# sitzikbs/Nesti-Net

Measured on AMD Instinct MI355X. Metric: normals/sec (whole node), synthetic 100k-pt clouds, higher is better.
Workload: dtype f16x8c

## Files before the change

nesti-net_amd/csrc/conv.hip:

```cpp
#include <type_traits>

#include "kernels.h"
#include "mma.h"

namespace nesti {
namespace {

constexpr int kThreads = 512;
constexpr int kABytes = kTileM * kRowBytes;
constexpr int kPoolStride = 272;

__device__ __forceinline__ int vox2(int b) { return b < 4 ? b : 11 - b; }
__device__ __forceinline__ int tile_row(int remap, int log2S, int wave, int mi, int l) {
  if (!remap) return wave * 64 + mi * 32 + l;
  if (remap == 2) return ((mi * 32 + l) << 3) + vox2(wave);
  const int c = wave & 3, s = 2 * (wave >> 2) + mi;
  const int q = (c - s) & 3;
  if (log2S == 3) return ((2 * s + (l >> 4)) << 6) + ((2 * q + ((l >> 3) & 1)) << 3) + (l & 7);
  return ((l >> 2) << 6) + (s << 4) + (q << 2) + (l & 3);
}
struct SwzKey {
  int m_lo, m_hi;
  __device__ __forceinline__ SwzKey(int remap, int log2S) {
    const bool pts = remap && log2S == 2;
// ... 486 lines not shown
      }
#pragma unroll
      for (int it = 0; it < 2; ++it) {
        const int item = it * kThreads + tid;
        const int orow = item >> 4, cg = item & 15;
        const int pt_l = orow >> (log2V - 3), cell = orow & (Vo - 1);
        const int cz = cell >> (2 * log2So), cy = (cell >> log2So) & (So - 1), cx = cell & (So - 1);
        const int base = (pt_l << log2V) + ((((2 * cz) << log2S) + 2 * cy) << log2S) + 2 * cx;
        float4 m = make_float4(-INFINITY, -INFINITY, -INFINITY, -INFINITY);
#pragma unroll
        for (int a = 0; a < 8; ++a) {
          const int row = base + ((a >> 2) << (2 * log2S)) + (((a >> 1) & 1) << log2S) + (a & 1);
          const float4 v = *reinterpret_cast<const float4*>(smem + row * kPoolStride + cg * 16);
          m.x = fmaxf(m.x, v.x); m.y = fmaxf(m.y, v.y); m.z = fmaxf(m.z, v.z); m.w = fmaxf(m.w, v.w);
        }
        const long long go = (r0 >> 3) + orow;
        if (go < (total_rows >> 3))
          store_out4<DT>(mp_b, go * p.mp_cstride, out_col0 + nh * 64 + cg * 4, m, out_esz, p.split);
      }
      __syncthreads();
    };
    mp_half(std::integral_constant<int, 0>{});
    if constexpr (TN == 128) mp_half(std::integral_constant<int, 1>{});
    return;
  }

  unsigned char* scratch = smem + wave * (32 * kPoolStride);
#pragma unroll
  for (int mi = 0; mi < 2; ++mi) {
#pragma unroll
    for (int nh = 0; nh < TN / 64; ++nh) {
#pragma unroll
      for (int n2 = 0; n2 < 2; ++n2) {
        const int ni = nh * 2 + n2;
        const int col = n2 * 32 + (lane & 31);
        const float bv = bias[ni * 32 + (lane & 31)];
#pragma unroll
        for (int r = 0; r < 16; ++r) {
          const int row = (r & 3) + 8 * (r >> 2) + 4 * khalf;
          *reinterpret_cast<float*>(scratch + row * kPoolStride + col * 4) = fmaxf(fmaf(acc[mi][ni][r], p.acc_scale, bv), act_floor);
        }
      }
      if (out_esz == 4) {
#pragma unroll
        for (int it = 0; it < 8; ++it) {
          const int row = it * 4 + (lane >> 4), cpos = lane & 15;
          const uint4 v = *reinterpret_cast<const uint4*>(scratch + row * kPoolStride + cpos * 16);
          const long long gr = r0 + tile_row(remap, log2S, wave, mi, row);
          if (gr < total_rows)
            *reinterpret_cast<uint4*>(out_b + (gr * p.out_cstride + out_col0 + nh * 64) * 4 + cpos * 16) = v;
        }
      } else {
        using E = Elem<DT == NESTI_F32 ? NESTI_BF16 : DT>;
#pragma unroll
        for (int it = 0; it < 4; ++it) {
          const int row = it * 8 + (lane >> 3), cpos = lane & 7;
          const float4 f0 = *reinterpret_cast<const float4*>(scratch + row * kPoolStride + cpos * 32);
          const float4 f1 = *reinterpret_cast<const float4*>(scratch + row * kPoolStride + cpos * 32 + 16);
          const long long gr = r0 + tile_row(remap, log2S, wave, mi, row);
          if (gr < total_rows) {
            store_act8<E>(out_b, gr * p.out_cstride, out_col0 + nh * 64 + cpos * 8, f0, f1, p.split);
            if (p.aux8_out && !second && p.x8_fmt != 6)
              store_aux8_8(reinterpret_cast<unsigned char*>(p.aux8_out) + gr * p.aux8_stride, n_local * TN + nh * 64 + cpos * 8, f0, f1,
                           aux_mul_lo, aux_mul_hi);
          }
        }
        if (p.aux8_out && !second && p.x8_fmt == 6) {
#pragma unroll
          for (int it = 0; it < 2; ++it) {
            const int row = it * 16 + (lane >> 2), c16 = lane & 3;
            const unsigned char* src = scratch + row * kPoolStride + c16 * 64;
            const long long gr = r0 + tile_row(remap, log2S, wave, mi, row);
            if (gr < total_rows)
              store_aux6_16(reinterpret_cast<unsigned char*>(p.aux8_out) + gr * p.aux8_stride, n_local * TN + nh * 64 + c16 * 16,
                            *reinterpret_cast<const float4*>(src), *reinterpret_cast<const float4*>(src + 16),
                            *reinterpret_cast<const float4*>(src + 32), *reinterpret_cast<const float4*>(src + 48));
          }
        }
      }
    }
  }
}

template <int DT, int TN, bool KPIPE, bool X3, bool WALK, bool X2 = false>
__global__ __launch_bounds__(kThreads) void conv_igemm_kernel(const ConvParams p) {
  if constexpr (!WALK) {
    conv_igemm_tile<DT, TN, KPIPE, X3, X2>(p, blockIdx.x, threadIdx.x);
  } else {
    const long long rows = (long long)live_points(p) << (3 * p.log2S);
    const unsigned m_live = (unsigned)((rows + kTileM - 1) / kTileM);
    const unsigned n_blocks = tile_rows8(m_live) * (unsigned)p.n_tiles;
    for (unsigned bid = blockIdx.x; bid < n_blocks; bid += gridDim.x) conv_igemm_tile<DT, TN, KPIPE, X3, X2>(p, bid, walk_trip(bid));
  }
}

template <int TN, bool KPIPE>
constexpr int lds_bytes() {
  constexpr size_t kPoolTile = (size_t)kTileM * kPoolStride + 16;
  constexpr size_t loop = KPIPE ? (size_t)2 * kABytes + 2 * TN * kRowBytes
                                : (size_t)kABytes + 4 * TN * kRowBytes + kRowBytes;
  static_assert(loop <= 163840 && kPoolTile <= 163840, "LDS budget");
  return (int)(loop > kPoolTile ? loop : kPoolTile);
}

template <int DT, int TN, bool KPIPE, bool X3>
int launch_one(const ConvParams& p, hipStream_t stream) {
  return launch_tiles<conv_igemm_kernel<DT, TN, KPIPE, X3, false>, conv_igemm_kernel<DT, TN, KPIPE, X3, true>>(
      p, lds_bytes<TN, KPIPE>(), kThreads, tile_rows8(p.m_tiles) * p.n_tiles, stream);
}
template <int DT, int TN>
int launch_one_x2(const ConvParams& p, hipStream_t stream) {
  return launch_tile_kernel<conv_igemm_kernel<DT, TN, true, false, false, true>>(p, lds_bytes<TN, true>(), kThreads,
                                                                                 tile_rows8(p.m_tiles) * p.n_tiles, stream);
}

template <int DT>
int launch_dt(const ConvParams& p, int TN, hipStream_t stream) {
  const bool kpipe = (p.n_taps == 1);
  if constexpr (DT != NESTI_F32) {
    if (p.x2) {
      if (!kpipe || p.x3native || p.walk) NESTI_FAIL("launch_conv: x2 is the filter pass's 1x1x1 / FC variant");
      if (TN == 128) return launch_one_x2<DT, 128>(p, stream);
      if (TN == 64) return launch_one_x2<DT, 64>(p, stream);
      NESTI_FAIL("launch_conv: unsupported N tile");
    }
    if (p.x3native) {
      if (TN == 128) return kpipe ? launch_one<DT, 128, true, true>(p, stream) : launch_one<DT, 128, false, true>(p, stream);
      if (TN == 64) return kpipe ? launch_one<DT, 64, true, true>(p, stream) : launch_one<DT, 64, false, true>(p, stream);
      NESTI_FAIL("launch_conv: unsupported N tile");
    }
  }
  if (p.x3native || p.x2) NESTI_FAIL("launch_conv: the pair / exact-weight K loops are for the 16-bit kernels");
  if (TN == 128) return kpipe ? launch_one<DT, 128, true, false>(p, stream) : launch_one<DT, 128, false, false>(p, stream);
  if (TN == 64) return kpipe ? launch_one<DT, 64, true, false>(p, stream) : launch_one<DT, 64, false, false>(p, stream);
  NESTI_FAIL("launch_conv: unsupported N tile");
}

}

int launch_conv(const ConvParams& p, int dtype, int TN, hipStream_t stream) {
  if (p.m_tiles <= 0 || p.n_tiles <= 0) return 0;
  if (p.pool_k > 1 && p.n_taps != 1) NESTI_FAIL("launch_conv: fused pooling needs a 1x1x1 layer");
  if (p.mp_mode != 0 && (p.log2S < 1 || !p.mp_out)) NESTI_FAIL("launch_conv: fused max-pool needs a volume >= 2^3 and an output");
  if (p.s_real && !(p.s_real == 3 && p.log2S == 2)) NESTI_FAIL("launch_conv: s_real is the 3^3 grid inside a 4^3 index space only");
  if (p.s_real && p.pool_k == 3) NESTI_FAIL("launch_conv: fused 3^3 avg-pool is not built for the embedded 3^3 volume");
  if (p.s_real && (p.mp_mode != 0 || p.mp_mode2 != 0)) NESTI_FAIL("launch_conv: the fused 2^3 max-pool does not apply to the 3^3 volume");
  if (p.mp_mode2 != 0 && (p.pool_k <= 1 || !p.mp_out || p.log2S < 1)) NESTI_FAIL("launch_conv: mp_mode2 belongs to a fused avg-pool half with a pooled output");
  if (p.pool_k > 1 && !((p.log2S == 3 && p.pool_k == 3) || (p.log2S == 2 && (p.pool_k == 2 || p.pool_k == 3)) ||
                        (p.log2S == 1 && p.pool_k == 2)))
    NESTI_FAIL("launch_conv: fused pooling supports (S,k) in {(8,3),(4,3),(4,2),(2,2)}");
  return with_elem_type(dtype, "launch_conv", [&](auto dt) { return launch_dt<decltype(dt)::value>(p, TN, stream); });
}

}
```

nesti-net_amd/csrc/kernels.h:

```cpp
#pragma once
#include <algorithm>
#include <type_traits>

#include "common.h"

namespace nesti {

constexpr unsigned kWalkGrid = 1024;

int launch_conv(const ConvParams& p, int dtype, int TN, hipStream_t stream);
int launch_conv8n(const ConvParams& p, int dtype, int k, hipStream_t stream);
int launch_conv4n(const ConvParams& p, int dtype, int k, hipStream_t stream);
int conv8_selftest();

__host__ __device__ __forceinline__ unsigned tile_rows8(unsigned m_tiles) { return (m_tiles + 7) / 8 * 8; }
template <class Params>
__device__ __forceinline__ int live_points(const Params& p) {
  int npts = p.npoints;
  if (p.npoints_ptr) npts = min(npts, *p.npoints_ptr);
  return npts;
}
struct TileId {
  int sub, m_tile;
};
__device__ __forceinline__ TileId tile_id(const unsigned bid, const int per_m) {
  const int xcd = bid & 7, grp = bid >> 3;
  return {grp % per_m, (grp / per_m) * 8 + xcd};
}
__device__ __forceinline__ int walk_trip(const unsigned bid) {
  if (bid != blockIdx.x) __syncthreads();
  int tid = threadIdx.x;
  asm volatile("" : "+v"(tid));
  return tid;
}

constexpr int kTapThreads = 512;
constexpr int kEpiStride = 144;
inline int check_tap_launch(const ConvParams& p, const char* who) {
  const std::string w(who);
  if (p.point_index) NESTI_FAIL(w + ": no input gather (k^3 layers never read the routed MuPS tensor)");
  if (p.pool_k > 1 || p.split_tile != p.n_tiles) NESTI_FAIL(w + ": no fused avg-pool / merged layers");
  if (p.mp_mode == 2) NESTI_FAIL(w + ": max-pool mode 2 is conv1's (a 1x1x1 layer)");
  if (p.mp_mode != 0 && !p.mp_out) NESTI_FAIL(w + ": fused max-pool needs an output");
  return 0;
}

template <auto Kernel>
int launch_tile_kernel(const ConvParams& p, int lds, unsigned threads, unsigned grid, hipStream_t stream) {
  constexpr int kMaxDevices = 64;
  static bool attr_set[kMaxDevices] = {};
  int dev = 0;
  NESTI_CHECK_HIP(hipGetDevice(&dev));
  if (dev < 0 || dev >= kMaxDevices || !attr_set[dev]) {
    NESTI_CHECK_HIP(hipFuncSetAttribute(reinterpret_cast<const void*>(Kernel), hipFuncAttributeMaxDynamicSharedMemorySize, lds));
    if (dev >= 0 && dev < kMaxDevices) attr_set[dev] = true;
  }
  hipLaunchKernelGGL(Kernel, dim3(grid), dim3(threads), lds, stream, p);
  NESTI_CHECK_HIP(hipGetLastError());
  return 0;
}
template <auto Kernel, auto WalkKernel>
int launch_tiles(const ConvParams& p, int lds, unsigned threads, unsigned n_blocks, hipStream_t stream) {
  if (!p.walk) return launch_tile_kernel<Kernel>(p, lds, threads, n_blocks, stream);
  return launch_tile_kernel<WalkKernel>(p, lds, threads, std::min(n_blocks, p.walk > 1 ? (unsigned)p.walk : kWalkGrid), stream);
}
template <class F>
int with_elem_type(int dtype, const char* who, F&& f) {
  if (dtype == NESTI_BF16) return f(std::integral_constant<int, NESTI_BF16>{});
  if (dtype == NESTI_F16) return f(std::integral_constant<int, NESTI_F16>{});
  if (dtype == NESTI_F32) return f(std::integral_constant<int, NESTI_F32>{});
  NESTI_FAIL(std::string(who) + ": unsupported dtype");
}

int launch_maxpool2(const PoolParams& p, int dtype, hipStream_t stream);
int launch_maxpool3s2(const PoolParams& p, int dtype, hipStream_t stream);

int launch_gate_finish(const float* logits, int lstride, int B, int E, float* probs,
                       int32_t* expert, int32_t* counts ,
                       int32_t* lists , hipStream_t stream);
constexpr int kMaxCascadeRounds = 24;
constexpr int kRoundCountsOff = 8, kTauEffOff = 40, kWidenUpperOff = 41, kWidenCountOff = 48, kWidenRoundsOff = 56;
static_assert(kRoundCountsOff + kMaxCascadeRounds <= kTauEffOff && kWidenRoundsOff + kMaxCascadeRounds <= 128, "fcounts layout");
int launch_gate_flag(const float* logits, int lstride, int B, int E, float tau, float widen, float* probs, int32_t* expert,
                     float* keep, int32_t* fcounts, int32_t* flag_list, int cap, int n_rounds, unsigned long long* cstat,
                     const unsigned long long* rstat, hipStream_t stream);
int launch_gate_widen(const float* keep, int B, int E, float widen, int32_t* fcounts, int32_t* flag_list, int cap, int n_rounds,
                      unsigned long long* cstat, hipStream_t stream);
int launch_gate_recheck(const float* logits, int lstride, const int32_t* flag_list, const int32_t* count_ptr, int cap, int E,
                        const float* keep, float* probs, int32_t* expert, unsigned long long* cstat, const int32_t* fcounts,
                        float widen, unsigned long long* rstat, hipStream_t stream);
int launch_stat_max_export(const unsigned long long* word, float* dst, hipStream_t stream);
int launch_stat_max_import(unsigned long long* word, const float* src, int n, hipStream_t stream);
int launch_round_counts(const int32_t* counts, int n_lists, int cap, int n_rounds, int32_t* out, hipStream_t stream);
// ... 18 lines not shown
```

nesti-net_amd/csrc/model.hip:

```cpp
#include <math.h>
#include <string.h>

#include <algorithm>
#include <map>
#include <memory>
#include <mutex>
#include <string>
#include <vector>

#include "kernels.h"
#include "plan.h"

#ifndef NESTI_GUARD_WALK_GRID
#define NESTI_GUARD_WALK_GRID 64
#endif
#ifndef NESTI_GUARD_LANES
#define NESTI_GUARD_LANES 2
#endif
#ifndef NESTI_GATE_WIDEN_WALK_GRID
#define NESTI_GATE_WIDEN_WALK_GRID 1
#endif
#ifndef NESTI_GUARD_WIDEN_WALK_GRID
#define NESTI_GUARD_WIDEN_WALK_GRID 8
#endif

namespace nesti {

static thread_local std::string g_error;
static bool g_experiment_mix = false;
void set_error(const std::string& msg) { g_error = msg; }

constexpr int kProfSlots = NESTI_PROF_PHASES * NESTI_PROF_CATEGORIES;
struct ProfState {
  bool on = false;
  int phase = NESTI_PHASE_INPUT;
  std::vector<hipEvent_t> pool;
  std::vector<std::pair<hipEvent_t, hipEvent_t>> spans[kProfSlots];
  double ms[kProfSlots] = {0};
  long long launches[kProfSlots] = {0};
};
static ProfState g_prof;
static std::mutex g_prof_mu;

static hipEvent_t prof_event() {
  if (!g_prof.pool.empty()) { hipEvent_t e = g_prof.pool.back(); g_prof.pool.pop_back(); return e; }
  hipEvent_t e = nullptr;
  (void)hipEventCreate(&e);
  return e;
}
static bool prof_capturing(hipStream_t st) {
  hipStreamCaptureStatus cs = hipStreamCaptureStatusNone;
  if (hipStreamIsCapturing(st, &cs) != hipSuccess) { (void)hipGetLastError(); return false; }
  return cs != hipStreamCaptureStatusNone;
}
void prof_phase(int phase) { if (g_prof.on) g_prof.phase = phase; }
int prof_begin(int cat, hipStream_t st) {
  if (!g_prof.on || prof_capturing(st)) return -1;
  std::lock_guard<std::mutex> lk(g_prof_mu);
  const int phase = (cat == NESTI_PROF_MUPS || cat == NESTI_PROF_PATCHES) ? NESTI_PHASE_INPUT : g_prof.phase;
  const int slot = phase * NESTI_PROF_CATEGORIES + cat;
  if (g_prof.spans[slot].size() >= (1u << 20)) return -1;
  hipEvent_t a = prof_event(), b = prof_event();
  (void)hipEventRecord(a, st);
  g_prof.spans[slot].push_back({a, b});
  return (slot << 20) | ((int)g_prof.spans[slot].size() - 1);
}
void prof_end(int, int token, hipStream_t st) {
  if (token < 0) return;
  std::lock_guard<std::mutex> lk(g_prof_mu);
  const int slot = token >> 20, idx = token & ((1 << 20) - 1);
  if (slot < kProfSlots && idx < (int)g_prof.spans[slot].size()) (void)hipEventRecord(g_prof.spans[slot][idx].second, st);
}
static void prof_collect() {
  std::lock_guard<std::mutex> lk(g_prof_mu);
  for (int c = 0; c < kProfSlots; ++c) {
    for (auto& sp : g_prof.spans[c]) {
      (void)hipEventSynchronize(sp.second);
      float ms = 0.f;
      if (hipEventElapsedTime(&ms, sp.first, sp.second) == hipSuccess) g_prof.ms[c] += ms;
      g_prof.launches[c] += 1;
      g_prof.pool.push_back(sp.first);
      g_prof.pool.push_back(sp.second);
    }
    g_prof.spans[c].clear();
  }
}

namespace {

struct PackedLayer : PackMeta {
  void* wpk = nullptr;
  float* bias = nullptr;
};

int upload(const PackedImage& img, PackedLayer* pl) {
  static_cast<PackMeta&>(*pl) = img;
  NESTI_CHECK_HIP(hipMalloc(&pl->wpk, img.w.size()));
  NESTI_CHECK_HIP(hipMemcpy(pl->wpk, img.w.data(), img.w.size(), hipMemcpyHostToDevice));
  NESTI_CHECK_HIP(hipMalloc((void**)&pl->bias, img.bias.size() * sizeof(float)));
  NESTI_CHECK_HIP(hipMemcpy(pl->bias, img.bias.data(), img.bias.size() * sizeof(float), hipMemcpyHostToDevice));
  return 0;
}

struct StatBlock {
  unsigned long long* dev = nullptr;
  StatBlock() = default;
  StatBlock(const StatBlock&) = delete;
  StatBlock& operator=(const StatBlock&) = delete;
  ~StatBlock() { if (dev) (void)hipFree(dev); }
  explicit operator bool() const { return dev != nullptr; }
  int alloc() { NESTI_CHECK_HIP(hipMalloc((void**)&dev, 64)); return reset(); }
  int reset() const { NESTI_CHECK_HIP(hipMemset(dev, 0, 64)); return 0; }
  int read(unsigned long long (&h)[8], int then_reset) const {
    memset(h, 0, sizeof(h));
    if (dev) NESTI_CHECK_HIP(hipMemcpy(h, dev, sizeof(h), hipMemcpyDeviceToHost));
    return dev && then_reset ? reset() : 0;
  }
};

}
}

struct nesti_model {
  nesti::Graph graph;
  int dtype = NESTI_BF16;
  std::map<std::pair<int, int>, nesti::PackedLayer> packed;
  const nesti::PackedLayer* packing(int form, int layer) const {
    auto it = packed.find({nesti::form_packing(form), layer});
    return it == packed.end() ? nullptr : &it->second;
  }
  const nesti::PackedLayer& main_packing(int layer) const {
    return *packing(nesti::act_planes(dtype) > 1 ? NESTI_DEBUG_FORM_PAIR : NESTI_DEBUG_FORM_PLAIN, layer);
  }
  bool cascade = false;
  nesti::Mode mode() const { return {graph, dtype, cascade}; }
  bool has_mix = false;
  int expert_mix = 0;
  int x8_mask = 0;
  int x8_fmt = 6;
  float x8_guard_thr = NESTI_X8_GUARD_DEFAULT;
  int x8_guard_walk = NESTI_GUARD_WALK_GRID;
  nesti::StatBlock gstat;
  static constexpr int kGuardLanes = NESTI_GUARD_LANES;
  struct GuardLane {
    hipStream_t gstream = nullptr;
    hipEvent_t gev_done[NESTI_MAX_EXPERTS] = {}, gev_join = nullptr;
    hipStream_t owner = nullptr;
    bool owned = false;
    std::mutex gmu;
  };
  mutable GuardLane glane[kGuardLanes];
  mutable std::mutex glane_mu;
  GuardLane* guard_lane(hipStream_t caller) const {
    std::lock_guard<std::mutex> lk(glane_mu);
    for (int i = 0; i < kGuardLanes; ++i) if (glane[i].owned && glane[i].owner == caller) return &glane[i];
    for (int i = 0; i < kGuardLanes; ++i) if (!glane[i].owned) { glane[i].owned = true; glane[i].owner = caller; return &glane[i]; }
    return &glane[0];
  }
  int gate_mix = 0;
  float tau = 0.25f;
  nesti::StatBlock cstat;
  bool reproducible = false;
  nesti::StatBlock rstat;
  unsigned long long* frozen() const { return reproducible ? rstat.dev : nullptr; }
  ~nesti_model() {
    for (auto& p : packed) {
      if (p.second.wpk) (void)hipFree(p.second.wpk);
      if (p.second.bias) (void)hipFree(p.second.bias);
    }
    for (auto& gl : glane) {
      if (gl.gstream) (void)hipStreamDestroy(gl.gstream);
      for (auto& ev : gl.gev_done) if (ev) (void)hipEventDestroy(ev);
      if (gl.gev_join) (void)hipEventDestroy(gl.gev_join);
    }
  }
};

namespace nesti {
namespace {

struct RunCtx {
  const nesti_model* m;
  Pass pass;
  int NB;
  const int32_t* npoints_ptr;
  const int32_t* point_index;
  hipStream_t stream;
  int walk;
};
RunCtx pass_ctx(const nesti_model* m, int tower, bool fast, int x8_mask, int NB, const int32_t* npoints_ptr, const int32_t* point_index,
                hipStream_t stream, int walk) {
  Pass ps;
  ps.tower = tower; ps.fast = fast; ps.x8_mask = x8_mask; ps.x8_fmt = m->x8_fmt;
  if (tower >= 0) ps.mix = m->expert_mix;
  else if (!m->cascade && m->gate_mix) { ps.mix = 1 << kGateMixBit; ps.zero_lo = m->gate_mix == 2; }
  return RunCtx{m, ps, NB, npoints_ptr, point_index, stream, walk};
}

int tower_ptrs(const RunCtx& rc, const Tower& T, const void* X0, unsigned char* ws, size_t ws_bytes, std::vector<unsigned char*>* ptr) {
  ptr->assign(T.bufs.size(), nullptr);
  (*ptr)[0] = (unsigned char*)X0;
  const Placement P = place_tower(T, rc.NB, pass_dtype(rc.pass.fast, rc.m->dtype));
  for (size_t i = 1; i < T.bufs.size(); ++i) (*ptr)[i] = ws + P.off[i];
  if (P.total > ws_bytes) NESTI_FAIL("workspace too small for this batch");
  return 0;
}

int run_op(const RunCtx& rc, const Tower& T, const Op& op, const std::vector<unsigned char*>& ptr) {
  const nesti_model* m = rc.m;
  const OpPlan plan = plan_op(m->graph, T, op, rc.pass, m->dtype);
  if (op.kind != Op::CONV) {
    PoolParams p = pool_params(T, op, plan, rc.NB);
    p.in = ptr[op.in_buf]; p.out = ptr[op.out_buf]; p.npoints_ptr = rc.npoints_ptr;
    const int tok = prof_begin(NESTI_PROF_POOL, rc.stream);
    const int rcp = op.kind == Op::MAX3 ? launch_maxpool3s2(p, plan.elem, rc.stream) : launch_maxpool2(p, plan.elem, rc.stream);
    prof_end(NESTI_PROF_POOL, tok, rc.stream);
    return rcp ? 1 : 0;
  }
  const LayerDesc& d = m->graph.layers[op.layer];
  const PackedLayer* pk = m->packing(plan.form.form, op.layer);
  if (!pk || pk->kind != plan.form.family)
    NESTI_FAIL("internal: layer " + d.scope + " is not packed for form " + std::to_string(plan.form.form) + " of this pass");
  ConvParams p = conv_params(m->graph, T, op, rc.pass, plan, *pk, plan.x8_sc_layer >= 0 ? m->main_packing(plan.x8_sc_layer).x8_sc : 0, rc.NB);
  p.in = ptr[op.in_buf]; p.out = ptr[op.out_buf]; p.wpk = pk->wpk; p.bias = pk->bias;
  p.npoints_ptr = rc.npoints_ptr; p.point_index = op.in_buf < 1 ? rc.point_index : nullptr;
  if (op.mp_buf >= 0) p.mp_out = ptr[op.mp_buf];
  if (p.x8) p.aux8_in = ptr[op.aux_in_buf];
  if (plan.form.producer) p.aux8_out = ptr[op.aux_out_buf];
  p.walk = rc.walk;
  const int cat = conv_category(d, *pk);
  const int tok = prof_begin(cat, rc.stream);
  const int rcv = pk->kind == 2   ? launch_conv8n(p, plan.elem, d.k, rc.stream)
                  : pk->kind == 3 ? launch_conv4n(p, plan.elem, d.k, rc.stream)
                                  : launch_conv(p, plan.elem, pk->TN, rc.stream);
  prof_end(cat, tok, rc.stream);
  return rcv ? 1 : 0;
}

int run_tower(const RunCtx& rc, const Tower& T, const void* X0, unsigned char* ws, size_t ws_bytes, float** out) {
  std::vector<unsigned char*> ptr;
  if (tower_ptrs(rc, T, X0, ws, ws_bytes, &ptr)) return 1;
  for (const Op& op : T.ops)
    if (run_op(rc, T, op, ptr)) return 1;
  *out = reinterpret_cast<float*>(ptr[T.out_buf]);
  return 0;
}

struct Arena {
  unsigned char* ws;
  int NB;
  WsLayout L;
  Arena(const nesti_model* m, void* ws_dev, int NB) : ws((unsigned char*)ws_dev), NB(NB), L(ws_layout(m->mode(), NB)) {}
  template <class T> T* at(size_t off) const { return reinterpret_cast<T*>(ws + off); }
  unsigned char* tower() const { return ws + L.tower; }
  size_t tower_size() const { return L.total - L.tower; }
};

int gate_cascade(const nesti_model* m, const void* X0, int B, const Arena& A, float* probs, int32_t* expert, int32_t* counts,
                 int32_t* lists, hipStream_t stream) {
  const int E = m->graph.cfg.n_experts;
  if (!expert) expert = A.at<int32_t>(A.L.expert);
  float* keep = A.at<float>(A.L.keep);
  int32_t* flag_list = A.at<int32_t>(A.L.flags);
  int32_t* fcounts = A.at<int32_t>(A.L.fcounts);
  const int lstride = m->graph.gate.bufs[m->graph.gate.out_buf].C;
  float* logits = nullptr;
  const RunCtx fast = pass_ctx(m, -1, true, 0, B, nullptr, nullptr, stream, 0);
  prof_phase(NESTI_PHASE_GATE);
  if (run_tower(fast, m->graph.gate, X0, A.tower(), A.tower_size(), &logits)) return 1;
  prof_phase(NESTI_PHASE_RECHECK);
  const int cap = std::min(cascade_cap(A.NB), B), rounds = (B + cap - 1) / cap;
  unsigned long long* rstat = m->frozen();
  if (launch_gate_flag(logits, lstride, B, E, m->tau, NESTI_GATE_WIDEN, probs, expert, keep, fcounts, flag_list, cap, rounds,
                       m->cstat.dev, rstat, stream))
    return 1;
  for (int pass = 0; pass <= (rstat ? 0 : NESTI_GATE_WIDEN_PASSES); ++pass) {
    if (pass >= 1 && launch_gate_widen(keep, B, E, NESTI_GATE_WIDEN, fcounts, flag_list, cap, rounds, m->cstat.dev, stream)) return 1;
    const int32_t* round_counts = fcounts + (pass == 0 ? kRoundCountsOff : kWidenRoundsOff);
    for (int r = 0; r < rounds; ++r) {
      const RunCtx exact = pass_ctx(m, -1, false, 0, cap, round_counts + r, flag_list + (size_t)r * cap, stream,
                                    pass >= 1 ? NESTI_GATE_WIDEN_WALK_GRID : r >= 1 ? 1 : 0);
      if (run_tower(exact, m->graph.gate, X0, A.tower(), A.tower_size(), &logits)) return 1;
      if (launch_gate_recheck(logits, lstride, flag_list + (size_t)r * cap, round_counts + r, cap, E, keep, probs, expert,
                              m->cstat.dev, fcounts, NESTI_GATE_WIDEN, rstat, stream))
        return 1;
    }
  }
  if (counts) return launch_route(expert, B, E, counts, lists, stream);
  return 0;
}

int gate_impl(const nesti_model* m, const void* X0, int B, const Arena& A, float* probs, int32_t* expert, int32_t* counts,
              int32_t* lists, hipStream_t stream) {
  if (m->cascade) return gate_cascade(m, X0, B, A, probs, expert, counts, lists, stream);
  const RunCtx rc = pass_ctx(m, -1, false, 0, B, nullptr, nullptr, stream, 0);
  float* logits = nullptr;
  prof_phase(NESTI_PHASE_GATE);
  if (run_tower(rc, m->graph.gate, X0, A.tower(), A.tower_size(), &logits)) return 1;
  const int lstride = m->graph.gate.bufs[m->graph.gate.out_buf].C;
  if (m->graph.cfg.arch == NESTI_ARCH_SWITCH)
    return launch_switch_finish(logits, lstride, B, 0.015f, probs, expert, counts, lists, stream);
  return launch_gate_finish(logits, lstride, B, m->graph.cfg.n_experts, probs, expert, counts, lists, stream);
}

constexpr int kGuardCountOff = 128, kGuardSlotOff = 140;
int experts_impl(const nesti_model* m, const void* X0, int B, const Arena& A, const int32_t* counts, const int32_t* lists, float* normals,
                 hipStream_t stream) {
  int32_t* ecounts = A.at<int32_t>(A.L.ecounts);
  int32_t* glist = m->graph.x8 ? A.at<int32_t>(A.L.glist) : nullptr;
  const int E = m->graph.cfg.n_experts;
  const int cap = std::min(expert_cap(A.NB), B), rounds = (B + cap - 1) / cap;
  prof_phase(NESTI_PHASE_EXPERTS);
  if (counts && launch_round_counts(counts, E, cap, rounds, ecounts, stream)) return 1;
  const size_t x0_row = mups_row_bytes(m->mode());
  const bool guard = counts && glist && m->x8_mask && m->gstat && m->x8_guard_thr >= 0.f;
  const int gcap = std::min(guard_cap(A.NB), B);
  float* gslot = guard ? reinterpret_cast<float*>(ecounts + kGuardSlotOff) : nullptr;
// ... 26 lines not shown
      float* out = nullptr;
      if (counts) {
        const int32_t* list = lists + (size_t)e * B + (size_t)r * cap;
        const int32_t* cnt = ecounts + e * rounds + r;
        const RunCtx rc = pass_ctx(m, e, false, m->x8_mask, cap, cnt, list, stream, r >= 1);
        if (run_tower(rc, T, X0, A.tower(), A.tower_size(), &out)) return 1;
        if (launch_scatter3(out, ostride, list, cnt, cap, normals, stream)) return 1;
      } else {
        const int take = std::min(cap, B - r * cap);
        const RunCtx rc = pass_ctx(m, e, false, m->x8_mask, take, nullptr, nullptr, stream, 0);
        if (run_tower(rc, T, (const unsigned char*)X0 + (size_t)r * cap * x0_row, A.tower(), A.tower_size(), &out)) return 1;
        if (launch_scatter3(out, ostride, nullptr, nullptr, take, normals + ((size_t)e * B + (size_t)r * cap) * 3, stream)) return 1;
      }
    }
    if (guard) {
      prof_phase(NESTI_PHASE_GUARD);
      if (side) {
        NESTI_CHECK_HIP(hipEventRecord(lane->gev_done[e], stream));
        NESTI_CHECK_HIP(hipStreamWaitEvent(lane->gstream, lane->gev_done[e], 0));
        if (guard_expert(e, lane->gstream, A.tower() + main_bytes, A.tower_size() - main_bytes, m->x8_guard_walk)) return 1;
      } else if (guard_expert(e, stream, A.tower(), A.tower_size(), m->x8_guard_walk)) {
        return 1;
      }
      prof_phase(NESTI_PHASE_EXPERTS);
    }
  }
  if (guard) {
    if (side) {
      NESTI_CHECK_HIP(hipEventRecord(lane->gev_join, lane->gstream));
      NESTI_CHECK_HIP(hipStreamWaitEvent(stream, lane->gev_join, 0));
      glk.unlock();
    }
    prof_phase(NESTI_PHASE_GUARD);
    for (int pass = 1; pass <= (rstat ? 0 : NESTI_X8_GUARD_WIDEN_PASSES); ++pass) {
      if (launch_x8_guard_begin(pass, m->x8_guard_thr, gscale, B, m->gstat.dev, gslot, nullptr, stream)) return 1;
      for (int e = 0; e < E; ++e)
        if (guard_expert(e, stream, A.tower(), A.tower_size(), NESTI_GUARD_WIDEN_WALK_GRID)) return 1;
    }
  }
  return 0;
}

}
}

using namespace nesti;

extern "C" {

const char* nesti_last_error(void) { return g_error.c_str(); }
const char* nesti_version(void) {
  return "nesti-hip 0.6 (gfx950)"
#ifdef NESTI_ATTRIBUTION
         " [measurement build: NESTI_ATTRIBUTION]"
#endif
#ifdef NESTI_EXPERIMENT_XW
         " [measurement build: NESTI_EXPERIMENT_XW]"
#endif
      ;
}

int nesti_mups_forward(const nesti_config_t* cfg, const float* points_dev, const int32_t* n_eff_dev, int B,
                       void* out_dev, int out_dtype, int out_cstride, void* stream) {
  if (B <= 0) return 0;
  if (!cfg || !points_dev || !n_eff_dev || !out_dev) NESTI_FAIL("nesti_mups_forward: null argument");
  const int tok = prof_begin(NESTI_PROF_MUPS, (hipStream_t)stream);
  const int rc = launch_mups(cfg, points_dev, n_eff_dev, B, out_dev, out_dtype, out_cstride, 0, (hipStream_t)stream);
  prof_end(NESTI_PROF_MUPS, tok, (hipStream_t)stream);
  return rc;
}

int nesti_model_create(const nesti_config_t* cfg, const nesti_tensor_t* tensors, int n_tensors, int dtype,
                       nesti_model_t** out) {
  if (!cfg || !tensors || !out) NESTI_FAIL("nesti_model_create: null argument");
  if (dtype != NESTI_F32 && dtype != NESTI_BF16 && dtype != NESTI_F16 && dtype != NESTI_BF16X3 && dtype != NESTI_F16X3 &&
      dtype != NESTI_F16X3C && dtype != NESTI_F16X8 && dtype != NESTI_F16X8C)
    NESTI_FAIL("nesti_model_create: bad dtype");
  if (dtype_cascade(dtype) && cfg->arch != NESTI_ARCH_EXPERTS)
    NESTI_FAIL("nesti_model_create: NESTI_F16X3C / NESTI_F16X8C is the two-stage gate of experts_n_est; use NESTI_F16X3 for the other models");
  if (dtype_x8(dtype) && (cfg->arch != NESTI_ARCH_EXPERTS || cfg->grid_n != 8))
    NESTI_FAIL("nesti_model_create: NESTI_F16X8 / NESTI_F16X8C (FP8 cross terms in the expert towers) is for experts_n_est on the 8^3 grid");
  std::unique_ptr<nesti_model> m(new nesti_model());
  m->cascade = dtype_cascade(dtype);
  const bool x8 = dtype_x8(dtype);
  dtype = main_dtype(dtype);
  m->dtype = dtype;
  if (build_graph(cfg, &m->graph, x8)) return 1;
  const TensorTable tt = tensor_table(tensors, n_tensors);
  bool any_conv8 = false;
  for (const LayerDesc& d : m->graph.layers) any_conv8 = any_conv8 || layer_kind(d, dtype) == 2;
  if (any_conv8 && conv8_selftest()) return 1;
  m->has_mix = g_experiment_mix && act_planes(dtype) > 1 && cfg->arch == NESTI_ARCH_EXPERTS && cfg->grid_n == 8;
  for (int t = -1; t < (int)m->graph.experts.size(); ++t) {
    std::vector<Pass> passes(1);
    if (m->cascade && t < 0) { passes.push_back(Pass()); passes.back().fast = true; }
    for (int fmt : {8, 6})
      if (x8 && t >= 0) { passes.push_back(Pass()); passes.back().x8_mask = 0xF; passes.back().x8_fmt = fmt; }
    if (m->has_mix) { passes.push_back(Pass()); passes.back().mix = t < 0 ? 1 << kGateMixBit : 0x3F; }
    for (Pass& ps : passes) {
      ps.tower = t;
      for (const Op& op : m->graph.tower(t).ops) {
        if (op.kind != Op::CONV) continue;
        const LayerDesc& d = m->graph.layers[op.layer];
        const LaunchForm f = launch_form(m->graph, op, ps, dtype);
        const int packing = form_packing(f.form);
        PackedLayer& pl = m->packed[{packing, op.layer}];
        PackedImage img;
        if (!pl.wpk && (pack_form(d, tt, packing, dtype, &img) || upload(img, &pl))) return 1;
        if (f.producer) pl.x8_sc = x8_activation_exponent(d, tt);
      }
    }
  }
  if (x8) {
    m->x8_mask = 0xF;
    if (m->gstat.alloc()) return 1;
    for (auto& gl : m->glane) {
      NESTI_CHECK_HIP(hipStreamCreateWithFlags(&gl.gstream, hipStreamNonBlocking));
      NESTI_CHECK_HIP(hipEventCreateWithFlags(&gl.gev_join, hipEventDisableTiming));
      for (int e = 0; e < cfg->n_experts; ++e) NESTI_CHECK_HIP(hipEventCreateWithFlags(&gl.gev_done[e], hipEventDisableTiming));
    }
  }
  if (m->cascade && m->cstat.alloc()) return 1;
  if ((m->cstat || m->gstat) && m->rstat.alloc()) return 1;
  NESTI_CHECK_HIP(hipDeviceSynchronize());
  *out = m.release();
  return 0;
}

void nesti_model_destroy(nesti_model_t* m) { delete m; }

int nesti_model_set_gate_margin(nesti_model_t* m, float tau) {
  if (!m || !m->cascade) NESTI_FAIL("nesti_model_set_gate_margin: not a NESTI_F16X3C model");
  if (!(tau >= 0.f)) NESTI_FAIL("nesti_model_set_gate_margin: tau must be >= 0");
  m->tau = tau;
  return 0;
}

int nesti_experiment_mix_enable(int on) {
  g_experiment_mix = on != 0;
  return 0;
}

int nesti_model_set_expert_mix(nesti_model_t* m, int mask) {
  if (!m) NESTI_FAIL("nesti_model_set_expert_mix: null model");
  if (mask && !m->has_mix) NESTI_FAIL("nesti_model_set_expert_mix: pair-mode experts_n_est models (8^3 grid) created after nesti_experiment_mix_enable(1) only");
  if (mask < 0 || mask >= (1 << 6)) NESTI_FAIL("nesti_model_set_expert_mix: mask has six bits");
  m->expert_mix = mask;
  return 0;
}

int nesti_model_set_x8_layers(nesti_model_t* m, int mask) {
  if (!m) NESTI_FAIL("nesti_model_set_x8_layers: null model");
  if (!m->graph.x8) NESTI_FAIL("nesti_model_set_x8_layers: not an NESTI_F16X8 / NESTI_F16X8C model");
  if (mask < 0 || mask > 0xF) NESTI_FAIL("nesti_model_set_x8_layers: mask has four bits (inception1 conv2 / conv3, inception2 conv2 / conv3)");
  m->x8_mask = mask;
  return 0;
}

int nesti_model_set_x8_format(nesti_model_t* m, int bits) {
  if (!m) NESTI_FAIL("nesti_model_set_x8_format: null model");
  if (!m->graph.x8) NESTI_FAIL("nesti_model_set_x8_format: not an NESTI_F16X8 / NESTI_F16X8C model");
  if (bits != 8 && bits != 6) NESTI_FAIL("nesti_model_set_x8_format: 8 (e4m3, one scale per layer) or 6 (e2m3, one scale per 16-channel block)");
  m->x8_fmt = bits;
  return 0;
}

// ... 458 lines not shown
```

Measured before the change: 51450.

## Add wide-N x3 pair conv kernel with 128x256 tiles and triple-buffered A

```diff
diff --git a/nesti-net_amd/csrc/conv.hip b/nesti-net_amd/csrc/conv.hip
--- a/nesti-net_amd/csrc/conv.hip
+++ b/nesti-net_amd/csrc/conv.hip
@@ -592,6 +592,300 @@
   }
 }
 
+constexpr int kWideRows = kTileM / 2;
+constexpr int kWideABuf = kWideRows * kRowBytes;
+constexpr int kWideBTile = 128 * kRowBytes;
+constexpr int kWideBBuf = 2 * kWideBTile;
+constexpr int kWideNA = 3, kWideNB = 2;
+constexpr int kWPieces = 4;
+static_assert(kWideNA * kWideABuf + kWideNB * kWideBBuf <= 163840 && kWideRows * kPoolStride + 16 <= 163840, "LDS budget");
+static_assert(kWideABuf == 8 * kWPieces * 1024 && kWideBBuf == 8 * kWPieces * 1024, "eight waves stage a whole A / B stage");
+
+template <int DT>
+__device__ __forceinline__ void conv_igemm_wide_tile(const ConvParams& p, const unsigned bid, const int tid_in) {
+  static_assert(DT != NESTI_F32, "the pair K loop is 16-bit");
+  extern __shared__ __attribute__((aligned(16))) unsigned char smem[];
+  constexpr int NI = 4;
+  unsigned char* As = smem;
+  unsigned char* Bs = smem + kWideNA * kWideABuf;
+
+  const int tid = tid_in, lane = tid & 63;
+  const int wave = __builtin_amdgcn_readfirstlane(tid >> 6);
+  const int wm = wave & 3, wn = wave >> 2;
+  const TileId t = tile_id(bid, p.n_tiles);
+  const int m_tile = t.m_tile, half = t.sub & 1, nt0 = t.sub & ~1;
+  if (m_tile >= p.m_tiles) return;
+  const int npts = live_points(p);
+  const int log2S = p.log2S, log2V = 3 * log2S;
+  const int S = 1 << log2S, V = 1 << log2V;
+  const long long total_rows = (long long)npts << log2V;
+  const long long r0 = (long long)m_tile * kTileM + half * kWideRows;
+  if (r0 >= total_rows) return;
+
+  long long a_off[kWPieces];
+#pragma unroll
+  for (int j = 0; j < kWPieces; ++j) {
+    const int row_l = (wave * kWPieces + j) * 8 + (lane >> 3);
+    const int slot = (lane & 7) ^ ((row_l >> 1) & 7);
+    const long long gr = r0 + row_l;
+    const long long grs = gr < total_rows ? gr : r0;
+    long long pt = grs >> log2V;
+    const long long vox = grs & (V - 1);
+    if (p.point_index) pt = p.point_index[pt];
+    a_off[j] = (((pt << log2V) + vox) * p.in_cstride + p.in_coff) * 2 + (slot & 3) * 16 + (slot >> 2) * (2 * kSplitGroup);
+  }
+  const unsigned char* in_b = reinterpret_cast<const unsigned char*>(p.in);
+  const unsigned char* w_pair = reinterpret_cast<const unsigned char*>(p.wpk) + (size_t)nt0 * p.n_chunks * kWideBTile;
+  const unsigned lds0 = (unsigned)(size_t)(lptr_t)smem;
+  auto stage_a = [&](int c, int a_buf) __attribute__((always_inline)) {
+#pragma unroll
+    for (int j = 0; j < kWPieces; ++j)
+      glds16(in_b + a_off[j] + (long long)(c >> 1) * (2 * kPairPlanes * kSplitGroup) + (c & 1) * 64,
+             lds0 + a_buf * kWideABuf + (wave * kWPieces + j) * 1024);
+  };
+  auto stage_b = [&](int c, int b_buf) __attribute__((always_inline)) {
+#pragma unroll
+    for (int q = 0; q < kWPieces; ++q) {
+      const int piece = wave * kWPieces + q;
+      glds16(w_pair + ((size_t)(piece >> 4) * p.n_chunks + c) * kWideBTile + (piece & 15) * 1024 + lane * 16,
+             lds0 + kWideNA * kWideABuf + b_buf * kWideBBuf + piece * 1024);
+    }
+  };
+
+  const int khalf = lane >> 5;
+  const int b_row = (lane & 31) * kRowBytes;
+  const int b_sw = ((lane & 31) >> 1) & 7;
+  int a_addr[2], a_sw[2];
+#pragma unroll
+  for (int mi = 0; mi < 2; ++mi) {
+    const int row = wm * 64 + mi * 32 + (lane & 31);
+    a_addr[mi] = row * kRowBytes;
+    a_sw[mi] = (row >> 1) & 7;
+  }
+
+  f32x16 acc[2][NI];
+#pragma unroll
+  for (int mi = 0; mi < 2; ++mi)
+#pragma unroll
+    for (int ni = 0; ni < NI; ++ni)
+#pragma unroll
+      for (int r = 0; r < 16; ++r) acc[mi][ni][r] = 0.f;
+
+  auto compute = [&](const unsigned char* Acur, const unsigned char* Bcur) __attribute__((always_inline)) {
+    uint4 ah[2], al[2], bh[NI], bl[NI];
+    auto ld_a = [&](int ks, int lo, uint4 (&f)[2]) __attribute__((always_inline)) {
+      const int slot = lo * 4 + ks * 2 + khalf;
+#pragma unroll
+      for (int mi = 0; mi < 2; ++mi) f[mi] = *reinterpret_cast<const uint4*>(Acur + a_addr[mi] + ((slot ^ a_sw[mi]) << 4));
+    };
+    auto ld_b = [&](int ks, int lo, uint4 (&f)[NI]) __attribute__((always_inline)) {
+      const int slot = lo * 4 + ks * 2 + khalf;
+#pragma unroll
+      for (int ni = 0; ni < NI; ++ni)
+        f[ni] = *reinterpret_cast<const uint4*>(Bcur + ni * 32 * kRowBytes + b_row + ((slot ^ b_sw) << 4));
+    };
+    auto mm = [&](const uint4 (&af)[2], const uint4 (&bf)[NI]) __attribute__((always_inline)) {
+#pragma unroll
+      for (int mi = 0; mi < 2; ++mi)
+#pragma unroll
+        for (int ni = 0; ni < NI; ++ni) mma<DT>(acc[mi][ni], af[mi], bf[ni]);
+    };
+    ld_a(0, 1, al);
+    ld_b(0, 0, bh);
+    ld_a(0, 0, ah);
+    ld_b(0, 1, bl);
+#pragma unroll
+    for (int ks = 0; ks < 2; ++ks) {
+      __builtin_amdgcn_sched_barrier(0);
+      mm(al, bh);
+      if (ks < 1) ld_a(ks + 1, 1, al);
+      __builtin_amdgcn_sched_barrier(0);
+      mm(ah, bh);
+      if (ks < 1) ld_b(ks + 1, 0, bh);
+      __builtin_amdgcn_sched_barrier(0);
+      mm(ah, bl);
+      if (ks < 1) {
+        ld_a(ks + 1, 0, ah);
+        ld_b(ks + 1, 1, bl);
+      }
+    }
+  };
+
+  const int n_chunks = p.n_chunks;
+  wait_vm0();
+  stage_a(0, 0);
+  stage_b(0, 0);
+  if (n_chunks > 1) stage_a(1, 1);
+  int sa = 0;
+  for (int c = 0; c < n_chunks; ++c) {
+    if (c + 1 < n_chunks) asm volatile("s_waitcnt vmcnt(%0)\n\ts_waitcnt lgkmcnt(0)" ::"n"(kWPieces) : "memory");
+    else asm volatile("s_waitcnt vmcnt(0)\n\ts_waitcnt lgkmcnt(0)" ::: "memory");
+    __builtin_amdgcn_s_barrier();
+    asm volatile("" ::: "memory");
+    if (c + 1 < n_chunks) stage_b(c + 1, (c + 1) & 1);
+    if (c + 2 < n_chunks) stage_a(c + 2, sa == 0 ? 2 : sa - 1);
+    compute(As + sa * kWideABuf, Bs + (c & 1) * kWideBBuf + wn * kWideBTile);
+    sa = sa == 2 ? 0 : sa + 1;
+  }
+  __syncthreads();
+
+  const int out_esz = p.out_f32 ? 4 : 2;
+  unsigned char* out_b = reinterpret_cast<unsigned char*>(p.out);
+  const float act_floor = p.relu ? 0.f : -INFINITY;
+  const float aux_mul_lo = __builtin_ldexpf(1.f, p.x8_sa), aux_mul_hi = __builtin_ldexpf(1.f, p.x8_sc);
+
+  if (p.mp_mode != 0) {
+    unsigned char* mp_b = reinterpret_cast<unsigned char*>(p.mp_out);
+    const int Vo = V >> 3, So = S >> 1, log2So = log2S - 1;
+    auto mp_pass = [&](auto PH) __attribute__((always_inline)) {
+      constexpr int ph = decltype(PH)::value, nh = ph & 1;
+      const int pcol0 = nt0 * 128 + ph * 64;
+      if (wn == (ph >> 1)) {
+#pragma unroll
+        for (int mi = 0; mi < 2; ++mi)
+#pragma unroll
+          for (int n2 = 0; n2 < 2; ++n2) {
+            const int ni = nh * 2 + n2;
+            const int col = n2 * 32 + (lane & 31);
+            const float bv = p.bias[pcol0 + col];
+#pragma unroll
+            for (int r = 0; r < 16; ++r) {
+              const int row = wm * 64 + mi * 32 + (r & 3) + 8 * (r >> 2) + 4 * khalf;
+              *reinterpret_cast<float*>(smem + row * kPoolStride + col * 4) = fmaxf(fmaf(acc[mi][ni][r], p.acc_scale, bv), act_floor);
+            }
+          }
+      }
+      __syncthreads();
+      if (p.mp_mode == 2) {
+#pragma unroll 4
+        for (int it = 0; it < kWideRows * 16 / kThreads; ++it) {
+          const int item = it * kThreads + tid;
+          const int row = item >> 4, cg = item & 15;
+          const long long gr = r0 + row;
+          if (gr < total_rows) {
+            const float4 v4 = *reinterpret_cast<const float4*>(smem + row * kPoolStride + cg * 16);
+            store_out4<DT>(out_b, gr * p.out_cstride, p.out_coff + pcol0 + cg * 4, v4, out_esz, p.split);
+            if (p.aux8_out && p.x8_fmt != 6)
+              store_aux8_4(reinterpret_cast<unsigned char*>(p.aux8_out) + gr * p.aux8_stride, pcol0 + cg * 4, v4.x, v4.y, v4.z, v4.w,
+                           aux_mul_lo, aux_mul_hi);
+          }
+        }
+        if (p.aux8_out && p.x8_fmt == 6) {
+#pragma unroll 2
+          for (int it = 0; it < kWideRows * 4 / kThreads; ++it) {
+            const int item = it * kThreads + tid;
+            const int row = item >> 2, c16 = item & 3;
+            const long long gr = r0 + row;
+            if (gr < total_rows) {
+              const unsigned char* src = smem + row * kPoolStride + c16 * 64;
+              store_aux6_16(reinterpret_cast<unsigned char*>(p.aux8_out) + gr * p.aux8_stride, pcol0 + c16 * 16,
+                            *reinterpret_cast<const float4*>(src), *reinterpret_cast<const float4*>(src + 16),
+                            *reinterpret_cast<const float4*>(src + 32), *reinterpret_cast<const float4*>(src + 48));
+            }
+          }
+        }
+      }
+      {
+        const int orow = tid >> 4, cg = tid & 15;
+        const int pt_l = orow >> (log2V - 3), cell = orow & (Vo - 1);
+        const int cz = cell >> (2 * log2So), cy = (cell >> log2So) & (So - 1), cx = cell & (So - 1);
+        const int base = (pt_l << log2V) + ((((2 * cz) << log2S) + 2 * cy) << log2S) + 2 * cx;
+        float4 m = make_float4(-INFINITY, -INFINITY, -INFINITY, -INFINITY);
+#pragma unroll
+        for (int a = 0; a < 8; ++a) {
+          const int row = base + ((a >> 2) << (2 * log2S)) + (((a >> 1) & 1) << log2S) + (a & 1);
+          const float4 v = *reinterpret_cast<const float4*>(smem + row * kPoolStride + cg * 16);
+          m.x = fmaxf(m.x, v.x); m.y = fmaxf(m.y, v.y); m.z = fmaxf(m.z, v.z); m.w = fmaxf(m.w, v.w);
+        }
+        const long long go = (r0 >> 3) + orow;
+        if (go < (total_rows >> 3))
+          store_out4<DT>(mp_b, go * p.mp_cstride, p.out_coff + pcol0 + cg * 4, m, out_esz, p.split);
+      }
+      __syncthreads();
+    };
+    mp_pass(std::integral_constant<int, 0>{});
+    mp_pass(std::integral_constant<int, 1>{});
+    mp_pass(std::integral_constant<int, 2>{});
+    mp_pass(std::integral_constant<int, 3>{});
+    return;
+  }
+
+  const int wcol0 = (nt0 + wn) * 128;
+  const float* bias = p.bias + wcol0;
+  unsigned char* scratch = smem + wave * (32 * kPoolStride);
+#pragma unroll
+  for (int mi = 0; mi < 2; ++mi) {
+#pragma unroll
+    for (int nh = 0; nh < 2; ++nh) {
+#pragma unroll
+      for (int n2 = 0; n2 < 2; ++n2) {
+        const int ni = nh * 2 + n2;
+        const int col = n2 * 32 + (lane & 31);
+        const float bv = bias[ni * 32 + (lane & 31)];
+#pragma unroll
+        for (int r = 0; r < 16; ++r) {
+          const int row = (r & 3) + 8 * (r >> 2) + 4 * khalf;
+          *reinterpret_cast<float*>(scratch + row * kPoolStride + col * 4) = fmaxf(fmaf(acc[mi][ni][r], p.acc_scale, bv), act_floor);
+        }
+      }
+      const long long gr0 = r0 + wm * 64 + mi * 32;
+      if (out_esz == 4) {
+#pragma unroll
+        for (int it = 0; it < 8; ++it) {
+          const int row = it * 4 + (lane >> 4), cpos = lane & 15;
+          const uint4 v = *reinterpret_cast<const uint4*>(scratch + row * kPoolStride + cpos * 16);
+          const long long gr = gr0 + row;
+          if (gr < total_rows)
+            *reinterpret_cast<uint4*>(out_b + (gr * p.out_cstride + p.out_coff + wcol0 + nh * 64) * 4 + cpos * 16) = v;
+        }
+      } else {
+        using E = Elem<DT>;
+#pragma unroll
+        for (int it = 0; it < 4; ++it) {
+          const int row = it * 8 + (lane >> 3), cpos = lane & 7;
+          const float4 f0 = *reinterpret_cast<const float4*>(scratch + row * kPoolStride + cpos * 32);
+          const float4 f1 = *reinterpret_cast<const float4*>(scratch + row * kPoolStride + cpos * 32 + 16);
+          const long long gr = gr0 + row;
+          if (gr < total_rows) {
+            store_act8<E>(out_b, gr * p.out_cstride, p.out_coff + wcol0 + nh * 64 + cpos * 8, f0, f1, p.split);
+            if (p.aux8_out && p.x8_fmt != 6)
+              store_aux8_8(reinterpret_cast<unsigned char*>(p.aux8_out) + gr * p.aux8_stride, wcol0 + nh * 64 + cpos * 8, f0, f1,
+                           aux_mul_lo, aux_mul_hi);
+          }
+        }
+        if (p.aux8_out && p.x8_fmt == 6) {
+#pragma unroll
+          for (int it = 0; it < 2; ++it) {
+            const int row = it * 16 + (lane >> 2), c16 = lane & 3;
+            const unsigned char* src = scratch + row * kPoolStride + c16 * 64;
+            const long long gr = gr0 + row;
+            if (gr < total_rows)
+              store_aux6_16(reinterpret_cast<unsigned char*>(p.aux8_out) + gr * p.aux8_stride, wcol0 + nh * 64 + c16 * 16,
+                            *reinterpret_cast<const float4*>(src), *reinterpret_cast<const float4*>(src + 16),
+                            *reinterpret_cast<const float4*>(src + 32), *reinterpret_cast<const float4*>(src + 48));
+          }
+        }
+      }
+    }
+  }
+}
+
+template <int DT, bool WALK>
+__global__ __launch_bounds__(kThreads) void conv_igemm_wide_kernel(const ConvParams p) {
+  auto tile = [&](const unsigned bid, const int tid) __attribute__((always_inline)) {
+    if (tile_id(bid, p.n_tiles).sub < p.split_tile) conv_igemm_wide_tile<DT>(p, bid, tid);
+    else conv_igemm_tile<DT, 128, true, true>(p, bid, tid);
+  };
+  if constexpr (!WALK) {
+    tile(blockIdx.x, threadIdx.x);
+  } else {
+    const long long rows = (long long)live_points(p) << (3 * p.log2S);
+    const unsigned m_live = (unsigned)((rows + kTileM - 1) / kTileM);
+    const unsigned n_blocks = tile_rows8(m_live) * (unsigned)p.n_tiles;
+    for (unsigned bid = blockIdx.x; bid < n_blocks; bid += gridDim.x) tile(bid, walk_trip(bid));
+  }
+}
+
 template <int DT, int TN, bool KPIPE, bool X3, bool WALK, bool X2 = false>
 __global__ __launch_bounds__(kThreads) void conv_igemm_kernel(const ConvParams p) {
   if constexpr (!WALK) {
@@ -625,7 +919,13 @@
 }
 
 template <int DT>
-int launch_dt(const ConvParams& p, int TN, hipStream_t stream) {
+int launch_one_wide(const ConvParams& p, hipStream_t stream) {
+  return launch_tiles<conv_igemm_wide_kernel<DT, false>, conv_igemm_wide_kernel<DT, true>>(p, lds_bytes<128, true>(), kThreads,
+                                                                                           tile_rows8(p.m_tiles) * p.n_tiles, stream);
+}
+
+template <int DT>
+int launch_dt(const ConvParams& p, int TN, hipStream_t stream, bool x3_wide) {
   const bool kpipe = (p.n_taps == 1);
   if constexpr (DT != NESTI_F32) {
     if (p.x2) {
@@ -635,6 +935,7 @@
       NESTI_FAIL("launch_conv: unsupported N tile");
     }
     if (p.x3native) {
+      if (x3_wide && kpipe && TN == 128 && p.split_tile >= 2 && p.split_tile % 2 == 0) return launch_one_wide<DT>(p, stream);
       if (TN == 128) return kpipe ? launch_one<DT, 128, true, true>(p, stream) : launch_one<DT, 128, false, true>(p, stream);
       if (TN == 64) return kpipe ? launch_one<DT, 64, true, true>(p, stream) : launch_one<DT, 64, false, true>(p, stream);
       NESTI_FAIL("launch_conv: unsupported N tile");
@@ -648,7 +949,7 @@
 
 }
 
-int launch_conv(const ConvParams& p, int dtype, int TN, hipStream_t stream) {
+int launch_conv(const ConvParams& p, int dtype, int TN, hipStream_t stream, bool x3_wide) {
   if (p.m_tiles <= 0 || p.n_tiles <= 0) return 0;
   if (p.pool_k > 1 && p.n_taps != 1) NESTI_FAIL("launch_conv: fused pooling needs a 1x1x1 layer");
   if (p.mp_mode != 0 && (p.log2S < 1 || !p.mp_out)) NESTI_FAIL("launch_conv: fused max-pool needs a volume >= 2^3 and an output");
@@ -659,7 +960,7 @@
   if (p.pool_k > 1 && !((p.log2S == 3 && p.pool_k == 3) || (p.log2S == 2 && (p.pool_k == 2 || p.pool_k == 3)) ||
                         (p.log2S == 1 && p.pool_k == 2)))
     NESTI_FAIL("launch_conv: fused pooling supports (S,k) in {(8,3),(4,3),(4,2),(2,2)}");
-  return with_elem_type(dtype, "launch_conv", [&](auto dt) { return launch_dt<decltype(dt)::value>(p, TN, stream); });
-}
-
-}
+  return with_elem_type(dtype, "launch_conv", [&](auto dt) { return launch_dt<decltype(dt)::value>(p, TN, stream, x3_wide); });
+}
+
+}
diff --git a/nesti-net_amd/csrc/kernels.h b/nesti-net_amd/csrc/kernels.h
--- a/nesti-net_amd/csrc/kernels.h
+++ b/nesti-net_amd/csrc/kernels.h
@@ -8,7 +8,7 @@
 
 constexpr unsigned kWalkGrid = 1024;
 
-int launch_conv(const ConvParams& p, int dtype, int TN, hipStream_t stream);
+int launch_conv(const ConvParams& p, int dtype, int TN, hipStream_t stream, bool x3_wide = true);
 int launch_conv8n(const ConvParams& p, int dtype, int k, hipStream_t stream);
 int launch_conv4n(const ConvParams& p, int dtype, int k, hipStream_t stream);
 int conv8_selftest();
diff --git a/nesti-net_amd/csrc/model.hip b/nesti-net_amd/csrc/model.hip
--- a/nesti-net_amd/csrc/model.hip
+++ b/nesti-net_amd/csrc/model.hip
@@ -1,4 +1,5 @@
 #include <math.h>
+#include <stdlib.h>
 #include <string.h>
 
 #include <algorithm>
@@ -138,6 +139,7 @@
   int expert_mix = 0;
   int x8_mask = 0;
   int x8_fmt = 6;
+  bool x3_wide = true;
   float x8_guard_thr = NESTI_X8_GUARD_DEFAULT;
   int x8_guard_walk = NESTI_GUARD_WALK_GRID;
   nesti::StatBlock gstat;
@@ -232,7 +234,7 @@
   const int tok = prof_begin(cat, rc.stream);
   const int rcv = pk->kind == 2   ? launch_conv8n(p, plan.elem, d.k, rc.stream)
                   : pk->kind == 3 ? launch_conv4n(p, plan.elem, d.k, rc.stream)
-                                  : launch_conv(p, plan.elem, pk->TN, rc.stream);
+                                  : launch_conv(p, plan.elem, pk->TN, rc.stream, m->x3_wide);
   prof_end(cat, tok, rc.stream);
   return rcv ? 1 : 0;
 }
@@ -425,6 +427,7 @@
     NESTI_FAIL("nesti_model_create: NESTI_F16X8 / NESTI_F16X8C (FP8 cross terms in the expert towers) is for experts_n_est on the 8^3 grid");
   std::unique_ptr<nesti_model> m(new nesti_model());
   m->cascade = dtype_cascade(dtype);
+  if (const char* e = getenv("NESTI_X3_WIDE")) m->x3_wide = e[0] != '0';
   const bool x8 = dtype_x8(dtype);
   dtype = main_dtype(dtype);
   m->dtype = dtype;
```

Measured after the change: 51570 (median of 6 runs). No clear change (+0.2%).
